# testingautomated-usi/simple-tip

Hardware: AMD Instinct MI355X
Metric: inputs_per_sec_prioritized (higher is better)
Workload: dtype bf16; 1 GPU; model=cifar10_resnet20, global_batch=20480, parallelism=dp1, train_ats=50000, at_width=4096, input_residency=hbm, scorers=gini+softmax-family+dsa+pc-lsa

## Files before the change

### simple_tip_amd/ops/hip/resnet_fused_device.h

```cpp

#pragma once

#include "tip_common.h"

#include <hip/hip_bf16.h>

using bf16 = __hip_bfloat16;
using short8 = __attribute__((ext_vector_type(8))) short;
using f32x4 = __attribute__((ext_vector_type(4))) float;

#ifndef TIP_SWZ_M
#define TIP_SWZ_M 0
#endif
TIP_DEV int swz(int u) {
  if (TIP_SWZ_M == 0) return u;
  return u ^ (((u >> 4) * TIP_SWZ_M) & 15);
}

#ifndef TIP_HALFPLANE
#define TIP_HALFPLANE 0
#endif

template <int H, int W, int C>
struct Img {
  static constexpr int UPP = C / 8;
#if TIP_HALFPLANE
  static constexpr int RS1 = W + 2;
  static constexpr int PLANE = (H + 2) * RS1;
  static constexpr int UNITS = UPP * PLANE;
  static constexpr int XSTEP = 1;
  static TIP_DEV int unit(int y, int x, int h) {
    return h * PLANE + y * RS1 + x;
  }
#else
  static constexpr int UNITS = (H + 2) * (W + 2) * UPP;
  static constexpr int XSTEP = UPP;
  static TIP_DEV int unit(int y, int x, int h) {
    return (y * (W + 2) + x) * UPP + h;
  }
#endif
};

TIP_DEV short8 lds_read_unit(const short* lds, int u) {
  return *reinterpret_cast<const short8*>(lds + swz(u) * 8);
}

TIP_DEV void lds_write_unit(short* lds, int u, short8 v) {
  *reinterpret_cast<short8*>(lds + swz(u) * 8) = v;
}

template <int H, int W, int C>
TIP_DEV void load_interior(short* lds, const short* __restrict__ gsrc) {
  using L = Img<H, W, C>;
  constexpr int UNITS = H * W * C / 8;
  constexpr int UPP = C / 8;
  for (int u = threadIdx.x; u < UNITS; u += blockDim.x) {
    const int p = u / UPP;
    const int h = u - p * UPP;
    const int y = p / W, x = p - y * W;
    const int lu = L::unit(y + 1, x + 1, h);
    short8 v = *reinterpret_cast<const short8*>(gsrc + (int64_t)u * 8);
    lds_write_unit(lds, lu, v);
  }
}

template <int H, int W, int C>
TIP_DEV void stage_plane(short* lds, const short* __restrict__ gsrc) {
  using L = Img<H, W, C>;
  const short8 zero = {0, 0, 0, 0, 0, 0, 0, 0};
  for (int u = threadIdx.x; u < L::UNITS; u += blockDim.x)
    lds_write_unit(lds, u, zero);
  __syncthreads();
  load_interior<H, W, C>(lds, gsrc);
}

template <int H, int W, int C, int COUT, bool TO_LDS, bool RESID, int STRIDE,
          bool INPLACE = false>
TIP_DEV void conv3x3(
    const short* __restrict__ in_lds,
    short* __restrict__ out_lds,
    short* __restrict__ gout,
    const short* __restrict__ rlds,
    const short* __restrict__ wpack,
    const float* __restrict__ bias) {
  constexpr int OH = H / STRIDE, OW = W / STRIDE;
  constexpr int K = 9 * C;
  constexpr int KSTEPS = (K + 31) / 32;
  constexpr int NPIX = OH * OW;
  constexpr int PIX_TILES = NPIX / 16;
  constexpr int COUT_TILES = COUT / 16;
  using In = Img<H, W, C>;
  using Out = Img<OH, OW, COUT>;
  static_assert(!INPLACE || (TO_LDS && RESID), "INPLACE is an LDS residual");

  const int lane = lane_id();
  const int wid = wave_id();
  const int j = lane & 15;
  const int g = lane >> 4;

  if constexpr (PIX_TILES <= 4 && (COUT_TILES % 2) == 0) {
    const int pt = wid;
    if (pt >= PIX_TILES) return;
    const int apix = pt * 16 + j;
    const int aoy = apix / OW, aox = apix - aoy * OW;
    const int abase = In::unit(aoy * STRIDE, aox * STRIDE, 0);
    for (int ct = 0; ct < COUT_TILES; ct += 2) {
      const short* wp0 = wpack + ((int64_t)ct * KSTEPS) * 64 * 8 + lane * 8;
      const short* wp1 = wp0 + (int64_t)KSTEPS * 64 * 8;
      f32x4 acc0 = {0.f, 0.f, 0.f, 0.f};
      f32x4 acc1 = {0.f, 0.f, 0.f, 0.f};
#pragma unroll
      for (int ks = 0; ks < KSTEPS; ++ks) {
        const int k0 = ks * 32 + g * 8;
        short8 a;
        if (k0 < K) {
          const int tap = k0 / C;
          const int ci = k0 & (C - 1);
          const int dy = (tap * 11) >> 5;
          const int dx = tap - dy * 3;
          a = lds_read_unit(in_lds, abase + In::unit(dy, dx, ci >> 3));
        } else {
          a = short8{0, 0, 0, 0, 0, 0, 0, 0};
        }
        const short8 b0 =
            *reinterpret_cast<const short8*>(wp0 + (int64_t)ks * 64 * 8);
        const short8 b1 =
            *reinterpret_cast<const short8*>(wp1 + (int64_t)ks * 64 * 8);
        acc0 = __builtin_amdgcn_mfma_f32_16x16x32_bf16(a, b0, acc0, 0, 0, 0);
        acc1 = __builtin_amdgcn_mfma_f32_16x16x32_bf16(a, b1, acc1, 0, 0, 0);
      }
#pragma unroll
      for (int half = 0; half < 2; ++half) {
        const int cout = (ct + half) * 16 + j;
        const float bs = bias[cout];
        const f32x4& acc = half ? acc1 : acc0;
        const int pix0 = pt * 16 + g * 4;
        const int oy = pix0 / OW, ox = pix0 - oy * OW;
        const int u0 = Out::unit(oy + 1, ox + 1, cout >> 3);
        const int e = cout & 7;
#pragma unroll
        for (int reg = 0; reg < 4; ++reg) {
          float v = acc[reg] + bs;
          if (RESID) {
            const short* rimg = INPLACE ? out_lds : rlds;
            const short* runit = rimg + swz(u0 + reg * Out::XSTEP) * 8;
            v += __bfloat162float(reinterpret_cast<const bf16*>(runit)[e]);
          }
          v = fmaxf(v, 0.f);
          const bf16 ov = __float2bfloat16(v);
          if (TO_LDS) {
            short* unit = out_lds + swz(u0 + reg * Out::XSTEP) * 8;
            reinterpret_cast<bf16*>(unit)[e] = ov;
          } else {
            reinterpret_cast<bf16*>(gout)[(int64_t)(pix0 + reg) * COUT + cout] =
                ov;
          }
        }
      }
    }
    return;
  }

  for (int ct = 0; ct < COUT_TILES; ++ct) {
    short8 bfrag[KSTEPS];
    {
      const short* wp = wpack + ((int64_t)ct * KSTEPS) * 64 * 8 + lane * 8;
#pragma unroll
      for (int ks = 0; ks < KSTEPS; ++ks)
        bfrag[ks] = *reinterpret_cast<const short8*>(wp + (int64_t)ks * 64 * 8);
    }
    const int cout = ct * 16 + j;
    const float bs = bias[cout];

    auto a_off = [&](int ks) {
      const int k0 = ks * 32 + g * 8;
      const int tap = k0 / C;
      const int ci = k0 & (C - 1);
      const int dy = (tap * 11) >> 5;
      const int dx = tap - dy * 3;
      return In::unit(dy, dx, ci >> 3);
    };
    auto a_base = [&](int pt) {
      const int apix = pt * 16 + j;
      const int aoy = apix / OW, aox = apix - aoy * OW;
      return In::unit(aoy * STRIDE, aox * STRIDE, 0);
    };
    auto epilogue = [&](int pt, const f32x4& acc) {
      const int pix0 = pt * 16 + g * 4;
      const int oy = pix0 / OW, ox = pix0 - oy * OW;
      const int u0 = Out::unit(oy + 1, ox + 1, cout >> 3);
      const int e = cout & 7;
#pragma unroll
      for (int reg = 0; reg < 4; ++reg) {
        float v = acc[reg] + bs;
        if (RESID) {
          const short* rimg = INPLACE ? out_lds : rlds;
          const short* runit = rimg + swz(u0 + reg * Out::XSTEP) * 8;
          v += __bfloat162float(reinterpret_cast<const bf16*>(runit)[e]);
        }
        v = fmaxf(v, 0.f);
        const bf16 ov = __float2bfloat16(v);
        if (TO_LDS) {
          short* unit = out_lds + swz(u0 + reg * Out::XSTEP) * 8;
          reinterpret_cast<bf16*>(unit)[e] = ov;
        } else {
          reinterpret_cast<bf16*>(gout)[(int64_t)(pix0 + reg) * COUT + cout] = ov;
        }
      }
    };

    int pt = wid;
    for (; pt + 4 < PIX_TILES; pt += 8) {
      const int b0 = a_base(pt), b1 = a_base(pt + 4);
      f32x4 acc0 = {0.f, 0.f, 0.f, 0.f};
      f32x4 acc1 = {0.f, 0.f, 0.f, 0.f};
#pragma unroll
      for (int ks = 0; ks < KSTEPS; ++ks) {
        const int k0 = ks * 32 + g * 8;
        short8 a0, a1;
        if (k0 < K) {
          const int off = a_off(ks);
          a0 = lds_read_unit(in_lds, b0 + off);
          a1 = lds_read_unit(in_lds, b1 + off);
        } else {
          a0 = short8{0, 0, 0, 0, 0, 0, 0, 0};
          a1 = a0;
        }
        acc0 = __builtin_amdgcn_mfma_f32_16x16x32_bf16(a0, bfrag[ks], acc0, 0, 0, 0);
        acc1 = __builtin_amdgcn_mfma_f32_16x16x32_bf16(a1, bfrag[ks], acc1, 0, 0, 0);
      }
      epilogue(pt, acc0);
      epilogue(pt + 4, acc1);
    }
    for (; pt < PIX_TILES; pt += 4) {
      const int b0 = a_base(pt);
      f32x4 acc = {0.f, 0.f, 0.f, 0.f};
#pragma unroll
      for (int ks = 0; ks < KSTEPS; ++ks) {
        const int k0 = ks * 32 + g * 8;
        short8 a;
        if (k0 < K) {
          a = lds_read_unit(in_lds, b0 + a_off(ks));
        } else {
          a = short8{0, 0, 0, 0, 0, 0, 0, 0};
        }
        acc = __builtin_amdgcn_mfma_f32_16x16x32_bf16(a, bfrag[ks], acc, 0, 0, 0);
      }
      epilogue(pt, acc);
    }
  }
}

template <int H, int W, int C, int COUT>
TIP_DEV void shortcut1x1_s2(
    const short* __restrict__ in_lds, short* __restrict__ rlds,
    const short* __restrict__ wpack, const float* __restrict__ bias) {
  constexpr int OH = H / 2, OW = W / 2;
  constexpr int KSTEPS = (C + 31) / 32;
  constexpr int NPIX = OH * OW;
  constexpr int PIX_TILES = NPIX / 16;
  constexpr int COUT_TILES = COUT / 16;
  using In = Img<H, W, C>;
  using Out = Img<OH, OW, COUT>;
  const int lane = lane_id();
  const int wid = wave_id();
  const int j = lane & 15;
  const int g = lane >> 4;
  for (int tile = wid; tile < PIX_TILES * COUT_TILES; tile += 4) {
    const int pt = tile % PIX_TILES;
    const int ct = tile / PIX_TILES;
    const int p0 = pt * 16;
    f32x4 acc = {0.f, 0.f, 0.f, 0.f};
    const short* wp = wpack + ((int64_t)ct * KSTEPS) * 64 * 8 + lane * 8;
    for (int ks = 0; ks < KSTEPS; ++ks) {
      const int k0 = ks * 32 + g * 8;
      short8 a = {0, 0, 0, 0, 0, 0, 0, 0};
      if (k0 < C) {
        const int pix = p0 + j;
        const int oy = pix / OW, ox = pix - oy * OW;
        const int iy = oy * 2 + 1, ix = ox * 2 + 1;
        a = lds_read_unit(in_lds, In::unit(iy, ix, k0 >> 3));
      }
      const short8 b = *reinterpret_cast<const short8*>(wp + (int64_t)ks * 64 * 8);
      acc = __builtin_amdgcn_mfma_f32_16x16x32_bf16(a, b, acc, 0, 0, 0);
    }
    const int cout = ct * 16 + j;
    const float bs = bias[cout];
    const int pix0 = p0 + g * 4;
    const int oy = pix0 / OW, ox = pix0 - oy * OW;
    const int u0 = Out::unit(oy + 1, ox + 1, cout >> 3);
#pragma unroll
    for (int reg = 0; reg < 4; ++reg) {
      short* unit = rlds + swz(u0 + reg * Out::XSTEP) * 8;
      reinterpret_cast<bf16*>(unit)[cout & 7] = __float2bfloat16(acc[reg] + bs);
    }
  }
}
```

Before: 5.158 million inputs/s.

## Transpose MFMA operands for vectorized epilogue and block over output-channel tiles

The MFMA operand order is swapped (weights as A, activations as B), so each lane's four accumulators now hold four consecutive output channels of one pixel instead of four pixels of one channel. The epilogue can then do one 8-byte packed bf16 load and store per lane, with vectorized bias and residual reads, replacing four scalar 2-byte accesses. The general conv path also processes two output-channel tiles per A-fragment read to halve LDS activation reads, and the 1x1 shortcut reuses its A fragments across all cout tiles. This costs more registers for the weight fragments and accumulators, and the small-tile fast path is apparently left unchanged.

```diff
diff --git a/simple_tip_amd/ops/hip/resnet_fused_device.h b/simple_tip_amd/ops/hip/resnet_fused_device.h
--- a/simple_tip_amd/ops/hip/resnet_fused_device.h
+++ b/simple_tip_amd/ops/hip/resnet_fused_device.h
@@ -72,6 +72,36 @@
     lds_write_unit(lds, u, zero);
   __syncthreads();
   load_interior<H, W, C>(lds, gsrc);
+}
+
+
+using f32x2 = __attribute__((ext_vector_type(2))) float;
+using bf16x2 = __attribute__((ext_vector_type(2))) __bf16;
+
+TIP_DEV unsigned pack2_bf16(float lo, float hi) {
+  const f32x2 v = {lo, hi};
+  return __builtin_bit_cast(unsigned, __builtin_convertvector(v, bf16x2));
+}
+
+TIP_DEV uint2 pack4_bf16(const f32x4& v) {
+  return uint2{pack2_bf16(v[0], v[1]), pack2_bf16(v[2], v[3])};
+}
+
+TIP_DEV void add4_bf16(f32x4& acc, const uint2 r) {
+  acc[0] += __uint_as_float(r.x << 16);
+  acc[1] += __uint_as_float(r.x & 0xffff0000u);
+  acc[2] += __uint_as_float(r.y << 16);
+  acc[3] += __uint_as_float(r.y & 0xffff0000u);
+}
+
+struct TilePix {
+  int oy, ox;
+};
+template <int OW>
+TIP_DEV TilePix tile_pix(int pt, int j) {
+  const int p = pt * 16 + j;
+  const int oy = p / OW;
+  return TilePix{oy, p - oy * OW};
 }
 
 template <int H, int W, int C, int COUT, bool TO_LDS, bool RESID, int STRIDE,
@@ -89,6 +119,7 @@
   constexpr int NPIX = OH * OW;
   constexpr int PIX_TILES = NPIX / 16;
   constexpr int COUT_TILES = COUT / 16;
+  constexpr int CTG = (COUT_TILES % 2) == 0 ? 2 : 1;
   using In = Img<H, W, C>;
   using Out = Img<OH, OW, COUT>;
   static_assert(!INPLACE || (TO_LDS && RESID), "INPLACE is an LDS residual");
@@ -98,7 +129,41 @@
   const int j = lane & 15;
   const int g = lane >> 4;
 
-  if constexpr (PIX_TILES <= 4 && (COUT_TILES % 2) == 0) {
+  auto read_a = [&](int base, int ks) {
+    const int k0 = ks * 32 + g * 8;
+    if (k0 >= K) return short8{0, 0, 0, 0, 0, 0, 0, 0};
+    const int tap = k0 / C;
+    const int ci = k0 & (C - 1);
+    const int dy = (tap * 11) >> 5;
+    const int dx = tap - dy * 3;
+    return lds_read_unit(in_lds, base + In::unit(dy, dx, ci >> 3));
+  };
+  auto a_base = [&](const TilePix& p) {
+    return In::unit(p.oy * STRIDE, p.ox * STRIDE, 0);
+  };
+  auto load_bias = [&](int ct) {
+    return *reinterpret_cast<const f32x4*>(bias + ct * 16 + g * 4);
+  };
+  auto epilogue = [&](int pt, const TilePix& p, int ct, const f32x4& acc,
+                      const f32x4& bs) {
+    const int c0 = ct * 16 + g * 4;
+    const int so = swz(Out::unit(p.oy + 1, p.ox + 1, c0 >> 3)) * 8 + (c0 & 7);
+    f32x4 v = acc + bs;
+    if (RESID) {
+      const short* rimg = INPLACE ? out_lds : rlds;
+      add4_bf16(v, *reinterpret_cast<const uint2*>(rimg + so));
+    }
+#pragma unroll
+    for (int r = 0; r < 4; ++r) v[r] = fmaxf(v[r], 0.f);
+    const uint2 o = pack4_bf16(v);
+    if (TO_LDS) {
+      *reinterpret_cast<uint2*>(out_lds + so) = o;
+    } else {
+      *reinterpret_cast<uint2*>(gout + (int64_t)(pt * 16 + j) * COUT + c0) = o;
+    }
+  };
+
+  if constexpr (PIX_TILES <= 4 && CTG == 2) {
     const int pt = wid;
     if (pt >= PIX_TILES) return;
     const int apix = pt * 16 + j;
@@ -161,92 +226,64 @@
     return;
   }
 
-  for (int ct = 0; ct < COUT_TILES; ++ct) {
-    short8 bfrag[KSTEPS];
-    {
-      const short* wp = wpack + ((int64_t)ct * KSTEPS) * 64 * 8 + lane * 8;
+  for (int ct = 0; ct < COUT_TILES; ct += CTG) {
+    short8 wfrag[CTG][KSTEPS];
+    f32x4 bs[CTG];
+#pragma unroll
+    for (int c = 0; c < CTG; ++c) {
+      const short* wp =
+          wpack + ((int64_t)(ct + c) * KSTEPS) * 64 * 8 + lane * 8;
 #pragma unroll
       for (int ks = 0; ks < KSTEPS; ++ks)
-        bfrag[ks] = *reinterpret_cast<const short8*>(wp + (int64_t)ks * 64 * 8);
-    }
-    const int cout = ct * 16 + j;
-    const float bs = bias[cout];
-
-    auto a_off = [&](int ks) {
-      const int k0 = ks * 32 + g * 8;
-      const int tap = k0 / C;
-      const int ci = k0 & (C - 1);
-      const int dy = (tap * 11) >> 5;
-      const int dx = tap - dy * 3;
-      return In::unit(dy, dx, ci >> 3);
-    };
-    auto a_base = [&](int pt) {
-      const int apix = pt * 16 + j;
-      const int aoy = apix / OW, aox = apix - aoy * OW;
-      return In::unit(aoy * STRIDE, aox * STRIDE, 0);
-    };
-    auto epilogue = [&](int pt, const f32x4& acc) {
-      const int pix0 = pt * 16 + g * 4;
-      const int oy = pix0 / OW, ox = pix0 - oy * OW;
-      const int u0 = Out::unit(oy + 1, ox + 1, cout >> 3);
-      const int e = cout & 7;
-#pragma unroll
-      for (int reg = 0; reg < 4; ++reg) {
-        float v = acc[reg] + bs;
-        if (RESID) {
-          const short* rimg = INPLACE ? out_lds : rlds;
-          const short* runit = rimg + swz(u0 + reg * Out::XSTEP) * 8;
-          v += __bfloat162float(reinterpret_cast<const bf16*>(runit)[e]);
-        }
-        v = fmaxf(v, 0.f);
-        const bf16 ov = __float2bfloat16(v);
-        if (TO_LDS) {
-          short* unit = out_lds + swz(u0 + reg * Out::XSTEP) * 8;
-          reinterpret_cast<bf16*>(unit)[e] = ov;
-        } else {
-          reinterpret_cast<bf16*>(gout)[(int64_t)(pix0 + reg) * COUT + cout] = ov;
-        }
-      }
-    };
+        wfrag[c][ks] =
+            *reinterpret_cast<const short8*>(wp + (int64_t)ks * 64 * 8);
+      bs[c] = load_bias(ct + c);
+    }
 
     int pt = wid;
     for (; pt + 4 < PIX_TILES; pt += 8) {
-      const int b0 = a_base(pt), b1 = a_base(pt + 4);
-      f32x4 acc0 = {0.f, 0.f, 0.f, 0.f};
-      f32x4 acc1 = {0.f, 0.f, 0.f, 0.f};
+      const TilePix p0 = tile_pix<OW>(pt, j), p1 = tile_pix<OW>(pt + 4, j);
+      const int b0 = a_base(p0), b1 = a_base(p1);
+      f32x4 acc0[CTG], acc1[CTG];
+#pragma unroll
+      for (int c = 0; c < CTG; ++c) {
+        acc0[c] = f32x4{0.f, 0.f, 0.f, 0.f};
+        acc1[c] = f32x4{0.f, 0.f, 0.f, 0.f};
+      }
 #pragma unroll
       for (int ks = 0; ks < KSTEPS; ++ks) {
-        const int k0 = ks * 32 + g * 8;
-        short8 a0, a1;
-        if (k0 < K) {
-          const int off = a_off(ks);
-          a0 = lds_read_unit(in_lds, b0 + off);
-          a1 = lds_read_unit(in_lds, b1 + off);
-        } else {
-          a0 = short8{0, 0, 0, 0, 0, 0, 0, 0};
-          a1 = a0;
+        const short8 a0 = read_a(b0, ks);
+        const short8 a1 = read_a(b1, ks);
+#pragma unroll
+        for (int c = 0; c < CTG; ++c) {
+          acc0[c] = __builtin_amdgcn_mfma_f32_16x16x32_bf16(
+              wfrag[c][ks], a0, acc0[c], 0, 0, 0);
+          acc1[c] = __builtin_amdgcn_mfma_f32_16x16x32_bf16(
+              wfrag[c][ks], a1, acc1[c], 0, 0, 0);
         }
-        acc0 = __builtin_amdgcn_mfma_f32_16x16x32_bf16(a0, bfrag[ks], acc0, 0, 0, 0);
-        acc1 = __builtin_amdgcn_mfma_f32_16x16x32_bf16(a1, bfrag[ks], acc1, 0, 0, 0);
-      }
-      epilogue(pt, acc0);
-      epilogue(pt + 4, acc1);
+      }
+#pragma unroll
+      for (int c = 0; c < CTG; ++c) {
+        epilogue(pt, p0, ct + c, acc0[c], bs[c]);
+        epilogue(pt + 4, p1, ct + c, acc1[c], bs[c]);
+      }
     }
     for (; pt < PIX_TILES; pt += 4) {
-      const int b0 = a_base(pt);
-      f32x4 acc = {0.f, 0.f, 0.f, 0.f};
+      const TilePix p0 = tile_pix<OW>(pt, j);
+      const int b0 = a_base(p0);
+      f32x4 acc[CTG];
+#pragma unroll
+      for (int c = 0; c < CTG; ++c) acc[c] = f32x4{0.f, 0.f, 0.f, 0.f};
 #pragma unroll
       for (int ks = 0; ks < KSTEPS; ++ks) {
-        const int k0 = ks * 32 + g * 8;
-        short8 a;
-        if (k0 < K) {
-          a = lds_read_unit(in_lds, b0 + a_off(ks));
-        } else {
-          a = short8{0, 0, 0, 0, 0, 0, 0, 0};
-        }
-        acc = __builtin_amdgcn_mfma_f32_16x16x32_bf16(a, bfrag[ks], acc, 0, 0, 0);
-      }
-      epilogue(pt, acc);
+        const short8 a = read_a(b0, ks);
+#pragma unroll
+        for (int c = 0; c < CTG; ++c)
+          acc[c] = __builtin_amdgcn_mfma_f32_16x16x32_bf16(
+              wfrag[c][ks], a, acc[c], 0, 0, 0);
+      }
+#pragma unroll
+      for (int c = 0; c < CTG; ++c) epilogue(pt, p0, ct + c, acc[c], bs[c]);
     }
   }
 }
@@ -266,33 +303,32 @@
   const int wid = wave_id();
   const int j = lane & 15;
   const int g = lane >> 4;
-  for (int tile = wid; tile < PIX_TILES * COUT_TILES; tile += 4) {
-    const int pt = tile % PIX_TILES;
-    const int ct = tile / PIX_TILES;
-    const int p0 = pt * 16;
-    f32x4 acc = {0.f, 0.f, 0.f, 0.f};
-    const short* wp = wpack + ((int64_t)ct * KSTEPS) * 64 * 8 + lane * 8;
+  for (int pt = wid; pt < PIX_TILES; pt += 4) {
+    const TilePix p = tile_pix<OW>(pt, j);
+    short8 a[KSTEPS];
+#pragma unroll
     for (int ks = 0; ks < KSTEPS; ++ks) {
       const int k0 = ks * 32 + g * 8;
-      short8 a = {0, 0, 0, 0, 0, 0, 0, 0};
-      if (k0 < C) {
-        const int pix = p0 + j;
-        const int oy = pix / OW, ox = pix - oy * OW;
-        const int iy = oy * 2 + 1, ix = ox * 2 + 1;
-        a = lds_read_unit(in_lds, In::unit(iy, ix, k0 >> 3));
-      }
-      const short8 b = *reinterpret_cast<const short8*>(wp + (int64_t)ks * 64 * 8);
-      acc = __builtin_amdgcn_mfma_f32_16x16x32_bf16(a, b, acc, 0, 0, 0);
-    }
-    const int cout = ct * 16 + j;
-    const float bs = bias[cout];
-    const int pix0 = p0 + g * 4;
-    const int oy = pix0 / OW, ox = pix0 - oy * OW;
-    const int u0 = Out::unit(oy + 1, ox + 1, cout >> 3);
-#pragma unroll
-    for (int reg = 0; reg < 4; ++reg) {
-      short* unit = rlds + swz(u0 + reg * Out::XSTEP) * 8;
-      reinterpret_cast<bf16*>(unit)[cout & 7] = __float2bfloat16(acc[reg] + bs);
-    }
-  }
-}
+      a[ks] = short8{0, 0, 0, 0, 0, 0, 0, 0};
+      if (k0 < C)
+        a[ks] = lds_read_unit(
+            in_lds, In::unit(p.oy * 2 + 1, p.ox * 2 + 1, k0 >> 3));
+    }
+#pragma unroll
+    for (int ct = 0; ct < COUT_TILES; ++ct) {
+      const short* wp = wpack + ((int64_t)ct * KSTEPS) * 64 * 8 + lane * 8;
+      f32x4 acc = {0.f, 0.f, 0.f, 0.f};
+#pragma unroll
+      for (int ks = 0; ks < KSTEPS; ++ks) {
+        const short8 b =
+            *reinterpret_cast<const short8*>(wp + (int64_t)ks * 64 * 8);
+        acc = __builtin_amdgcn_mfma_f32_16x16x32_bf16(b, a[ks], acc, 0, 0, 0);
+      }
+      const int c0 = ct * 16 + g * 4;
+      const int so =
+          swz(Out::unit(p.oy + 1, p.ox + 1, c0 >> 3)) * 8 + (c0 & 7);
+      const f32x4 v = acc + *reinterpret_cast<const f32x4*>(bias + c0);
+      *reinterpret_cast<uint2*>(rlds + so) = pack4_bf16(v);
+    }
+  }
+}
```

Result: faster. 5.325 million inputs/s (median of 6 runs) (+3.2%).
